# tnwei/waternet

Measured on NVIDIA H100. Metric: images/sec at 1080p batch16 (preprocess + gated-fusion forward, uint8 in -> uint8 out), higher is better.
Workload: dtype bf16 + fp8 corrections (v = hi + lo: hi x hi in bf16, both correction terms of the heavy layers as one e4m3 MMA; fp32 accumulate; 3-term bf16 elsewhere)

## Files before the change

### waternet_b200/csrc/common.cuh

```cuda
#pragma once

#include <cuda_runtime.h>
#include <stdint.h>
#include <stdio.h>

#include "../../include/waternet_b200.h"
#include "tiling.cuh"

namespace wn {

void set_error(const char* fmt, ...);

#define WN_CUDA(call)                                                                   \
  do {                                                                                  \
    cudaError_t err__ = (call);                                                         \
    if (err__ != cudaSuccess) {                                                         \
      wn::set_error("%s:%d: %s -> %s", __FILE__, __LINE__, #call, cudaGetErrorString(err__)); \
      return WN_E_CUDA;                                                                 \
    }                                                                                   \
  } while (0)

#define WN_LAUNCH_CHECK(h)   \
  do {                       \
    (h)->launches++;         \
// ... 144 lines not shown
};
struct FwdOpts {
  int scheme = 0;
  int dbg_layer = -1;
  float* dbg_dst = nullptr;
  bool packed = false;
  bool hi_only = false;
  const int* run_if = nullptr;
  uint8_t* out_u8 = nullptr;
  PeerOut peers = {};
  int stack = kStackAll;
  bool refiner_l1 = false;
  const TileGeom* tiles = nullptr;
  long long win0 = 0;
  const RaggedWindow* rwin = nullptr;
};
int umma_forward_layers(wn_handle* h, const float* const in[4], const int64_t st[4][4], float* out, int n,
                        int height, int width, const FwdBuffers& b, cudaStream_t stream,
                        const FwdOpts& opts = FwdOpts());
int umma_debug_layer(wn_handle* h, const float* const in[4], const int64_t in_strides[4][4], int n,
                     int height, int width, int layer, float* dst, void* workspace,
                     size_t workspace_bytes, cudaStream_t stream, int scheme = 0);
int umma_pack_weights(wn_handle* h, const float* const* params, cudaStream_t stream);
void umma_free(wn_handle* h);
size_t umma_forward_workspace_bytes(int n, int h, int w);
int umma_chunk_images(const wn_handle* h, int n, int height, int width);
int umma_forward(wn_handle* h, const float* const in[4], const int64_t in_strides[4][4], float* out,
                 int n, int height, int width, void* workspace, size_t workspace_bytes,
                 cudaStream_t stream, int scheme = 0, int stack = kStackAll, float* refined = nullptr);
size_t umma_forward_tiled_workspace_bytes(int n, int h, int w, int tile_h, int tile_w, long long max_pass_pixels,
// ... 51 lines not shown
```

### waternet_b200/csrc/conv_umma.cu

```cuda
#include "umma_conv.cuh"

namespace wn {

struct PackInArgs {
  const float* p[4];
  long long s[4][4];
};
enum PackForm { kPackImages = 0, kPackWindows = 1, kPackFlag = 2 };
template <int FORM = kPackImages>
__global__ void __launch_bounds__(256) pack_inputs_kernel(PackInArgs a, uint4* __restrict__ out, int H, int W,
                                                          int* __restrict__ exact_flag, TileGeom tiles, long long win0) {
  const int pix = blockIdx.x * 256 + threadIdx.x;
  const int hw = FORM == kPackWindows ? tiles.win_h * tiles.win_w : H * W;
  bool exact = true;
  if (pix < hw) {
    int n = blockIdx.y, y, x;
    if constexpr (FORM == kPackWindows) {
      const TileWindow t = tile_window(tiles, win0 + blockIdx.y);
      const int wy = pix / tiles.win_w;
      n = t.img;
      y = t.ys + wy;
      x = t.xs + (pix - wy * tiles.win_w);
    } else {
      y = pix / W;
// ... 59 lines not shown
static constexpr UmmaLayerSpec kSpecs[kNumUmmaLayers] = {
    {7, 16, 224, kEpiAct, 0, 1, 1, 0, false, 1, 1},
    {5, 128, 128, kEpiAct, 0, 1, 5, 1, true, 1, 1},
    {3, 128, 128, kEpiAct, 0, 1, 3, 2, true, 1, 1},
    {1, 128, 64, kEpiAct, 1, 1, 1, 3, false, 1, 1},
    {7, 64, 64, kEpiAct, 1, 1, 7, 4, true, 2, 1},
    {5, 64, 64, kEpiAct, 1, 1, 5, 5, true, 2, 1},
    {3, 64, 64, kEpiAct, 1, 1, 9, 6, true, 2, 1},
    {3, 64, 16, kEpiSigmoid, 1, 1, 9, 7, false, 1, 1},
    {5, 96, 32, kEpiAct, 1, 3, 5, 9, true, 1, 1},
    {3, 96, 16, kEpiGate, 1, 1, 9, 10, false, 1, 1},
    {7, 16, 96, kEpiAct, 0, 1, 1, 8, false, 1, 1}};

static_assert(kSpecs[kC2].f8 == kSpecs[kR2].f8, "L1 writes one format for both of its consumers");
static constexpr bool writes_f8(int li) { return li < kR3 && li != kC8 && kSpecs[li + 1].f8; }

static __global__ void __launch_bounds__(256)
mirror_u8_kernel(const uint8_t* __restrict__ src, PeerOut peers, size_t bytes, const int* __restrict__ run_if) {
  if (run_if && *run_if == 0) return;
  const size_t stride = (size_t)gridDim.x * blockDim.x, i0 = (size_t)blockIdx.x * blockDim.x + threadIdx.x;
#pragma unroll
  for (int k = 0; k < WN_MAX_PEERS; k++) {
    if (k >= peers.n) continue;
    uint8_t* dst = peers.p[k];
    const size_t vecs = (((reinterpret_cast<uintptr_t>(src) | reinterpret_cast<uintptr_t>(dst)) & 15) == 0) ? bytes / 16 : 0;
    for (size_t i = i0; i < vecs; i += stride) reinterpret_cast<uint4*>(dst)[i] = reinterpret_cast<const uint4*>(src)[i];
    for (size_t i = vecs * 16 + i0; i < bytes; i += stride) dst[i] = src[i];
  }
}
int mirror_u8(wn_handle* h, const uint8_t* src, const PeerOut& peers, size_t bytes, const int* run_if, cudaStream_t stream) {
// ... 109 lines not shown
  if (cap <= 0 || cap > kDefaultChunkPixels) cap = kDefaultChunkPixels;
  long long per = (long long)h * w;
  long long nb = cap / (per > 0 ? per : 1);
  if (nb < 1) nb = 1;
  return nb < n ? (int)nb : n;
}
int umma_chunk_images(const wn_handle* h, int n, int height, int width) {
  return umma_chunk(h ? h->chunk_pixels : 0, n, height, width);
}

size_t umma_forward_workspace_bytes(int n, int h, int w) {
  const size_t nb = (size_t)umma_chunk(0, n, h, w);
  return nb * h * w * kUmmaBytesPerPixel + nb * h * 64 + 4096;
}

template <int LI, bool RAG>
static int launch_layer_as(wn_handle* h, bool f8, void* in_base, ConvArgs a, cudaStream_t stream) {
  constexpr UmmaLayerSpec s = kSpecs[LI];
  constexpr bool R = RAG && s.epi != kEpiSigmoid;
  const UmmaWeights* u = h->umma;
  constexpr int GW = s.npad / s.ng;
  if (f8) {
    constexpr int FMT = (s.f8 ? kFmtIn8 : 0) | (writes_f8(LI) ? kFmtOut8 : 0);
    if constexpr ((FMT & kFmtOut8) != 0) a.f8_overflow = u->overflow_dev;
    if constexpr (s.f8) a.f8_scale = u->scale8[LI] + 1;
    return launch_conv<s.ks, s.cinpad, GW, s.epi, (s.f8 ? 0 : s.concat), s.nblk, s.tps, FMT, R, s.mw, s.ng>(
        h, s.slot, s.f8 ? u->stages8[LI] : u->stages[LI], u->bias[LI], in_base, a, stream);
  }
  return launch_conv<s.ks, s.cinpad, GW, s.epi, s.concat, s.nblk, s.tps, 0, R, s.mw, s.ng>(
      h, s.slot, u->stages[LI], u->bias[LI], in_base, a, stream);
}
template <int LI>
static int launch_layer(wn_handle* h, bool f8, void* in_base, ConvArgs a, cudaStream_t stream) {
  return a.rwin ? launch_layer_as<LI, true>(h, f8, in_base, a, stream)
                : launch_layer_as<LI, false>(h, f8, in_base, a, stream);
}

__global__ void decode_planes_kernel(const uint4* __restrict__ src, float* __restrict__ dst, int planes_half, int hw,
                                     int f8) {
  const int n = blockIdx.z, plane = blockIdx.y;
  const int pix = blockIdx.x * blockDim.x + threadIdx.x;
  if (pix >= hw) return;
  const uint4 h4 = src[((size_t)n * 2 * planes_half + plane) * hw + pix];
  if (f8) {
    const uint4 l4 = src[((size_t)n * 2 * planes_half + planes_half + 2 * (plane >> 1)) * hw + pix];
    const uint32_t hs[4] = {h4.x, h4.y, h4.z, h4.w}, ls[4] = {l4.x, l4.y, l4.z, l4.w};
#pragma unroll
    for (int j = 0; j < 8; j++) {
      const float hi = __uint_as_float(((hs[j >> 1] >> ((j & 1) * 16)) & 0xffffu) << 16);
      const int byte = (plane & 1) * 8 + j;
// ... 76 lines not shown
    act(b.r[1], 96, nullptr, 0);
    rc = launch_conv<s.ks, s.cinpad, s.npad, s.epi, s.concat, s.nblk, s.tps, 0, false, s.mw, s.ng>(
        h, s.slot, h->umma->stages[kRL1], h->umma->bias[kRL1], b.act0, a, stream);
    if (rc) return rc;
  } else {
    act(b.a[1], 128, b.r[1], b.r[1] ? 96 : 0);
    if ((rc = launch_layer<kL1>(h, f8, b.act0, a, stream))) return rc;
  }
  a.skip_lo = nullptr;
  a.a_hi_only = 0;
  if (dump(kL1)) return WN_OK;
  if (want_cmg) {
    act(b.a[2], 128, nullptr, 0);
    if ((rc = launch_layer<kC2>(h, f8, b.a[1], a, stream))) return rc;
    if (dump(kC2)) return WN_OK;
    act(b.a[3], 128, nullptr, 0);
    if ((rc = launch_layer<kC3>(h, f8, b.a[2], a, stream))) return rc;
    if (dump(kC3)) return WN_OK;
    act(b.a[4], 64, nullptr, 0);
    if ((rc = launch_layer<kC4>(h, f8, b.a[3], a, stream))) return rc;
    if (dump(kC4)) return WN_OK;
    act(b.a[5], 64, nullptr, 0);
    if ((rc = launch_layer<kC5>(h, f8, b.a[4], a, stream))) return rc;
    if (dump(kC5)) return WN_OK;
    act(b.a[6], 64, nullptr, 0);
    if ((rc = launch_layer<kC6>(h, f8, b.a[5], a, stream))) return rc;
    if (dump(kC6)) return WN_OK;
    act(b.a[7], 64, nullptr, 0);
    if ((rc = launch_layer<kC7>(h, f8, b.a[6], a, stream))) return rc;
    if (dump(kC7)) return WN_OK;
    const bool dump_maps = dbg_layer == kSpecs[kC8].slot;
    a.out_f32 = dump_maps ? dbg_dst : b.cm;
    if ((rc = launch_layer<kC8>(h, f8, b.a[7], a, stream))) return rc;
    if (dump_maps) return WN_OK;
  }
// ... 16 lines not shown

static FwdBuffers carve(void* workspace, int n, int H, int W) {
  const size_t px = (size_t)n * H * W;
  uint8_t* ws = (uint8_t*)(((uintptr_t)workspace + 1023) / 1024 * 1024);
  uint4* cmgAB[2];
  uint4* refAB[2];
  FwdBuffers b;
  memset(&b, 0, sizeof(b));
  b.act0 = (uint4*)ws;     ws += px * 64;
  cmgAB[0] = (uint4*)ws;   ws += px * 512;
  cmgAB[1] = (uint4*)ws;   ws += px * 512;
  refAB[0] = (uint4*)ws;   ws += px * 384;
  refAB[1] = (uint4*)ws;   ws += px * 384;
  b.cm = (float*)ws;       ws += px * 12;
  b.exact_flag = (int*)(((uintptr_t)ws + 255) / 256 * 256);
  for (int l = 1; l <= 7; l++) b.a[l] = cmgAB[(l - 1) & 1];
  b.r[1] = refAB[0];
  b.r[2] = refAB[1];
  return b;
}

static int umma_pass(wn_handle* h, const float* const in[4], const int64_t st[4][4], float* out, int n, int H, int W,
                     const FwdBuffers& b, cudaStream_t stream, FwdOpts o) {
  int rc = umma_forward_layers(h, in, st, out, n, H, W, b, stream, o);
  if (rc || o.scheme != 1 || o.dbg_layer >= 0) return rc;
  o.scheme = 0;
  o.packed = true;
  o.run_if = h->umma->overflow_dev;
  Timing* timing = h->timing;
  h->timing = nullptr;
  rc = umma_forward_layers(h, in, st, out, n, H, W, b, stream, o);
  h->timing = timing;
  return rc;
}

int umma_debug_layer(wn_handle* h, const float* const in[4], const int64_t in_strides[4][4], int n, int H, int W,
                     int layer, float* dst, void* workspace, size_t workspace_bytes, cudaStream_t stream, int scheme) {
  if (!h->umma || umma_chunk(0, n, H, W) != n || workspace_bytes < umma_forward_workspace_bytes(n, H, W)) {
    set_error("debug layer dump: weights not packed, batch too large for one pass or workspace too small");
    return WN_E_WORKSPACE;
  }
  int rc = get_encoder();
  if (rc) return rc;
  FwdOpts o;
  o.scheme = scheme;
  o.dbg_layer = layer;
  o.dbg_dst = dst;
  return umma_forward_layers(h, in, in_strides, nullptr, n, H, W, carve(workspace, n, H, W), stream, o);
}

static int effective_scheme(wn_handle* h, int scheme) {
  return (scheme == 1 && *h->umma->overflow_host) ? 0 : scheme;
}
static int mirror_overflow(wn_handle* h, int scheme, cudaStream_t stream) {
  if (scheme == 1)
    WN_CUDA(cudaMemcpyAsync(h->umma->overflow_host, h->umma->overflow_dev, sizeof(int), cudaMemcpyDeviceToHost, stream));
  return WN_OK;
}

int umma_forward(wn_handle* h, const float* const in[4], const int64_t in_strides[4][4], float* out, int n, int H,
                 int W, void* workspace, size_t workspace_bytes, cudaStream_t stream, int scheme, int stack,
                 float* refined) {
// ... 298 lines not shown
```

### waternet_b200/csrc/umma_conv.cuh

```cuda
#pragma once

#include <cuda.h>
#include <cuda_bf16.h>

#include "common.cuh"
#include "wgmma_ops.cuh"

namespace wn {

__device__ __forceinline__ uint32_t smem_u32(const void* p) {
  return (uint32_t)__cvta_generic_to_shared(p);
}
__device__ __forceinline__ void mbar_init(uint64_t* bar, uint32_t count) {
  asm volatile("mbarrier.init.shared::cta.b64 [%0], %1;" ::"r"(smem_u32(bar)), "r"(count));
}
__device__ __forceinline__ void mbar_wait(uint64_t* bar, uint32_t parity) {
  for (uint32_t it = 0; it < (1u << 26); it++) {
    uint32_t done;
    asm volatile(
        "{\n\t.reg .pred p;\n\t"
        "mbarrier.try_wait.parity.shared::cta.b64 p, [%1], %2;\n\t"
        "selp.u32 %0, 1, 0, p;\n\t}"
        : "=r"(done)
        : "r"(smem_u32(bar)), "r"(parity)
// ... 42 lines not shown
  uint16_t v;
  asm("cvt.rn.satfinite.e4m3x2.f32 %0, %1, %2;" : "=h"(v) : "f"(f1), "f"(f0));
  return v;
}

enum Epilogue { kEpiAct = 0, kEpiSigmoid = 1, kEpiGate = 2, kEpiDgrad = 3 };

constexpr int kTileH = 16;
constexpr int kThreads = 320;
constexpr int kWarpA = 8, kWarpB = 9;
constexpr int kConsumerWarps = 8;
constexpr int kStageLd = 36;

constexpr int kFmtIn8 = 1, kFmtOut8 = 2;
template <int KS, int CIN_PAD, int NPAD, int CONCAT = 0, int NBLK = 1, int TPS = 1, int FMT = 0, int MW = 1,
          int NG = 1>
struct UmmaCfg {
  static constexpr bool F8IN = (FMT & kFmtIn8) != 0;
  static constexpr bool DUAL = CONCAT != 0;
  static constexpr int TILE_W = 8 * MW;
  static constexpr int HALO_W = TILE_W + KS - 1, HALO_H = kTileH + KS - 1;
  static constexpr int NCHUNK = CIN_PAD / 16;
  static constexpr int PLANE_BYTES = HALO_W * HALO_H * 16;
  static constexpr int A_STAGE = (4 * PLANE_BYTES + 1023) / 1024 * 1024;
  static constexpr int B_TAP = NPAD * 64;
  static constexpr int B_STAGE = TPS * B_TAP;
  static_assert((KS * KS) % TPS == 0, "taps per weight stage must divide the filter");
  static constexpr int NSTAGE_PER_CHUNK = KS * KS / TPS;
  static constexpr int STAGING = 2 * 64 * kStageLd * 4;
  static constexpr int BUDGET = 227 * 1024 - 1024 - 2048 - STAGING;
  static constexpr int NA_WANT = NCHUNK == 1 ? 2 : KS == 1 ? 6 : 3;
  static constexpr int NB_FIT = (BUDGET - NA_WANT * A_STAGE) / B_STAGE;
  static constexpr int NB = NB_FIT > 8 ? 8 : NB_FIT < 2 ? 2 : NB_FIT;
  static constexpr int NA_FIT = (BUDGET - NB * B_STAGE) / A_STAGE;
  static constexpr int NA = NA_FIT > NA_WANT ? NA_WANT : NA_FIT;
  static_assert(!F8IN || !CONCAT, "fp8 corrections: the [hi | second part] weight layout");
  static constexpr int CPB = NCHUNK / NBLK;
  static constexpr int BLK_COLS = DUAL ? 2 * NPAD : NPAD;
  static constexpr int COLS = NBLK * BLK_COLS;
  static constexpr int ACC = COLS / 2;
  static constexpr int ACC8 = F8IN ? ACC : 1;
  static constexpr int SMEM_BYTES = NA * A_STAGE + NB * B_STAGE + STAGING + 2048 + 1024;
  static_assert(NA >= 1, "halo tile does not fit in shared memory");
  static_assert(NCHUNK % NBLK == 0, "chunks must split evenly over the diagonal blocks");
  static_assert(NPAD % 16 == 0 && (DUAL ? 2 : 1) * NPAD <= 256, "invalid wgmma N");
  static_assert(MW == 1 || MW == 2, "one or two m64 blocks per warpgroup");
  static_assert(NG == 1 || NBLK == 1, "column groups of a block-diagonal layer");
  static_assert(MW * (ACC + (F8IN ? ACC8 : 0)) <= 128, "accumulators do not fit in registers");
  static constexpr size_t GROUP_BYTES = (size_t)NCHUNK * NSTAGE_PER_CHUNK * B_STAGE;
};

struct ActDst {
  uint4* base;
  int planes_half;
};

struct ConvArgs {
  const uint8_t* wpk;
  const float* bias;
  int N, H, W;
  int in_planes_half;
  int tiles_x, tiles_y;
  ActDst dst0, dst1;
  int split_c;
// ... 1 lines not shown
  float* out_f32;
  const float* cm;
  uint8_t* out_u8;
  const int* skip_lo;
  int a_hi_only;
  float* refined_out;
  const uint4* mask_base;
  int mask_planes_half;
  const float* f8_scale;
  int* f8_overflow;
  const int* run_if;
  int tiled;
  long long win0;
  TileGeom tiles;
  const RaggedWindow* rwin;
};

__device__ __forceinline__ uint32_t pack_bf16x2(__nv_bfloat16 a, __nv_bfloat16 b) {
  return (uint32_t)__bfloat16_as_ushort(a) | ((uint32_t)__bfloat16_as_ushort(b) << 16);
}
__device__ __forceinline__ void split_bf16x2(float f0, float f1, uint32_t& hi, uint32_t& lo) {
  const __nv_bfloat162 h = __floats2bfloat162_rn(f0, f1);
  hi = *reinterpret_cast<const uint32_t*>(&h);
  const float h0 = __uint_as_float(hi << 16), h1 = __uint_as_float(hi & 0xffff0000u);
  const __nv_bfloat162 l = __floats2bfloat162_rn(f0 - h0, f1 - h1);
  lo = *reinterpret_cast<const uint32_t*>(&l);
}

template <int EPI, bool OUT8, bool RAG = false>
__device__ __forceinline__ void epilogue16(const ConvArgs& g, const float* s_bias, const float* f, int ch, int n,
// ... 116 lines not shown
        if (out_f32) {
#pragma unroll
          for (int c = 0; c < 3; c++) out_f32[oo + c * ohw] = v[c];
        }
        if (out_u8) {
          uint8_t* q = out_u8 + o8;
#pragma unroll
          for (int c = 0; c < 3; c++) q[c] = (uint8_t)(int)__fmul_rn(fminf(fmaxf(v[c], 0.0f), 1.0f), 255.0f);
        }
      }
    }
  }
}

template <int KS, int CIN_PAD, int NPAD, int EPI, int CONCAT, int NBLK, int TPS, int FMT = 0, bool RAG = false,
          int MW = 1, int NG = 1>
__global__ void __launch_bounds__(kThreads, 1)
conv_umma_kernel(const __grid_constant__ CUtensorMap tmap_in, const ConvArgs g) {
  using C = UmmaCfg<KS, CIN_PAD, NPAD, CONCAT, NBLK, TPS, FMT, MW, NG>;
  constexpr bool F8IN = C::F8IN, DUAL = C::DUAL, OUT8 = (FMT & kFmtOut8) != 0;
  static_assert(!OUT8 || EPI == kEpiAct, "fp8 planes are written by the activation epilogue only");
  static_assert(!RAG || EPI == kEpiAct || EPI == kEpiGate, "ragged passes mask activations and store the gate");
  if (g.run_if != nullptr && *reinterpret_cast<const volatile int*>(g.run_if) == 0) return;
  extern __shared__ uint8_t smem_raw[];
  uint8_t* smem = reinterpret_cast<uint8_t*>((reinterpret_cast<uintptr_t>(smem_raw) + 1023) & ~(uintptr_t)1023);
  uint8_t* a_stages = smem;
  uint8_t* b_stages = smem + C::NA * C::A_STAGE;
  float* staging = reinterpret_cast<float*>(b_stages + C::NB * C::B_STAGE);
  uint8_t* tail = reinterpret_cast<uint8_t*>(staging) + C::STAGING;
  uint64_t* a_full = reinterpret_cast<uint64_t*>(tail);
  uint64_t* a_empty = a_full + C::NA;
  uint64_t* b_full = a_empty + C::NA;
  uint64_t* b_empty = b_full + C::NB;
  float* s_bias = reinterpret_cast<float*>(tail + 512);
  static_assert((2 * 6 + 2 * 8) * 8 <= 512 && NG * NBLK * NPAD * 4 <= 2048 - 512, "barrier / bias area");

  const int tid = threadIdx.x, warp = tid >> 5, lane = tid & 31;
  const int num_tiles = g.tiles_x * g.tiles_y * g.N * NG;
  if (tid == 0) {
    for (int i = 0; i < C::NA; i++) { mbar_init(&a_full[i], 1); mbar_init(&a_empty[i], kConsumerWarps); }
    for (int i = 0; i < C::NB; i++) { mbar_init(&b_full[i], 1); mbar_init(&b_empty[i], kConsumerWarps); }
    asm volatile("fence.mbarrier_init.release.cluster;" ::: "memory");
  }
  for (int i = tid; i < NG * NBLK * NPAD; i += kThreads) s_bias[i] = g.bias[i];
  __syncthreads();

  if (warp == kWarpA) {
    if (lane == 0) {
      int stage = 0;
      uint32_t phase = 0;
      for (int tile = blockIdx.x; tile < num_tiles; tile += gridDim.x) {
        const int pt = tile / NG;
        const int n = pt / (g.tiles_x * g.tiles_y);
        const int rem = pt - n * g.tiles_x * g.tiles_y;
        const int ty = rem / g.tiles_x, tx = rem - ty * g.tiles_x;
        const int x0 = tx * C::TILE_W - KS / 2, y0 = ty * kTileH - KS / 2;
        for (int c = 0; c < C::NCHUNK; c++) {
          mbar_wait(&a_empty[stage], phase ^ 1);
          uint8_t* dst = a_stages + stage * C::A_STAGE;
          mbar_expect_tx(&a_full[stage], (g.a_hi_only ? 2 : 4) * C::PLANE_BYTES);
          tma_load_5d(dst, &tmap_in, &a_full[stage], 0, x0, y0, 2 * c, n);
          if (!g.a_hi_only)
            tma_load_5d(dst + 2 * C::PLANE_BYTES, &tmap_in, &a_full[stage], 0, x0, y0, g.in_planes_half + 2 * c, n);
          if (++stage == C::NA) { stage = 0; phase ^= 1; }
        }
      }
    }
    return;
  }
  if (warp == kWarpB) {
    if (lane == 0) {
      int stage = 0;
      uint32_t phase = 0;
      for (int tile = blockIdx.x; tile < num_tiles; tile += gridDim.x) {
        const uint8_t* wpk = g.wpk + (size_t)(tile % NG) * C::GROUP_BYTES;
        for (int it = 0; it < C::NCHUNK * C::NSTAGE_PER_CHUNK; it++) {
          mbar_wait(&b_empty[stage], phase ^ 1);
          mbar_expect_tx(&b_full[stage], C::B_STAGE);
          bulk_load(b_stages + stage * C::B_STAGE, wpk + (size_t)it * C::B_STAGE, C::B_STAGE, &b_full[stage]);
          if (++stage == C::NB) { stage = 0; phase ^= 1; }
        }
      }
    }
    return;
  }

// ... 63 lines not shown
        wg_wait<1>();
        release();
        pend_b = bstage;
        if (tg == C::NSTAGE_PER_CHUNK - 1) pend_a = astage;
        if (++bstage == C::NB) { bstage = 0; bphase ^= 1; }
      }
      if (++astage == C::NA) { astage = 0; aphase ^= 1; }
    }
    wg_wait<0>();
    release();

    const int pt = tile / NG, c0 = (tile % NG) * NPAD;
    const int n = pt / (g.tiles_x * g.tiles_y);
    const int rem = pt - n * g.tiles_x * g.tiles_y;
    const int ty = rem / g.tiles_x, tx = rem - ty * g.tiles_x;
    float* stg = staging + wg * 64 * kStageLd;
    const int frow = (warp & 3) * 16 + (lane >> 2), fcol = (lane & 3) * 2;
    const int r = wtid & 63, half = wtid >> 6;
    const int m = wg * 64 + r;
    const int gy = ty * kTileH + (m >> 3);
    constexpr int NCH = NBLK * NPAD;
#pragma unroll
    for (int mb = 0; mb < MW; mb++) {
      const int gx = tx * C::TILE_W + mb * 8 + (m & 7);
      const bool inside = gx < g.W && gy < g.H;
      bool valid = true;
      if constexpr (RAG) valid = gx < g.rwin[n].vw && gy < g.rwin[n].vh;
#pragma unroll
      for (int ch0 = 0; ch0 < NCH; ch0 += 32) {
#pragma unroll
        for (int j = 0; j < 4; j++) {
          const int ch = ch0 + 8 * j;
          if (ch < NCH) {
            const int col = NBLK > 1 ? (ch / NPAD) * C::BLK_COLS + ch % NPAD : ch;
            float v[4];
#pragma unroll
            for (int k = 0; k < 4; k++) {
              v[k] = acc[mb][col / 2 + k];
              if constexpr (DUAL) v[k] += acc[mb][(col + NPAD) / 2 + k];
              if constexpr (F8IN) v[k] = (v[k] + acc8[mb][col / 2 + k]) * dscale;
            }
            float* s = stg + frow * kStageLd + 8 * j + fcol;
            *reinterpret_cast<float2*>(s) = make_float2(v[0], v[1]);
            *reinterpret_cast<float2*>(s + 8 * kStageLd) = make_float2(v[2], v[3]);
          }
        }
        wg_bar(1 + wg);
        const int cb = ch0 + 16 * half;
        if (cb < NCH && inside) {
          float f[16];
          const float4* s = reinterpret_cast<const float4*>(stg + r * kStageLd + 16 * half);
#pragma unroll
          for (int q = 0; q < 4; q++) {
            const float4 x = s[q];
            f[4 * q] = x.x; f[4 * q + 1] = x.y; f[4 * q + 2] = x.z; f[4 * q + 3] = x.w;
          }
          epilogue16<EPI, OUT8, RAG>(g, s_bias, f, c0 + cb, n, gx, gy, valid);
        }
        wg_bar(1 + wg);
      }
    }
  }
}

static __global__ void scatter_weights_kernel(const float* __restrict__ src, float* __restrict__ dense, int co, int ci,
                                       int kk, int cinpad, int row_off, int split, int base0, int base1,
                                       float divisor) {
  const int total = co * ci * kk;
  for (int i = blockIdx.x * blockDim.x + threadIdx.x; i < total; i += gridDim.x * blockDim.x) {
    int t = i % kk;
    int c = (i / kk) % ci;
    int o = i / (kk * ci);
// ... 112 lines not shown
  cuuint64_t strides[4] = {16, (cuuint64_t)W * 16, (cuuint64_t)H * W * 16, (cuuint64_t)planes_total * H * W * 16};
  cuuint32_t box[5] = {8, (cuuint32_t)halo_w, (cuuint32_t)halo_h, 2, 1};
  cuuint32_t estr[5] = {1, 1, 1, 1, 1};
  CUresult r = g_encode(tm, CU_TENSOR_MAP_DATA_TYPE_BFLOAT16, 5, base, dims, strides, box, estr,
                        CU_TENSOR_MAP_INTERLEAVE_NONE, CU_TENSOR_MAP_SWIZZLE_NONE, CU_TENSOR_MAP_L2_PROMOTION_L2_128B,
                        CU_TENSOR_MAP_FLOAT_OOB_FILL_NONE);
  if (r != CUDA_SUCCESS) {
    set_error("cuTensorMapEncodeTiled failed with %d (planes=%d N=%d H=%d W=%d box=%dx%d)", (int)r, planes_total, N, H,
              W, halo_w, halo_h);
    return WN_E_CUDA;
  }
  return WN_OK;
}

template <int KS, int CIN_PAD, int NPAD, int EPI, int CONCAT = 0, int NBLK = 1, int TPS = 1, int FMT = 0,
          bool RAG = false, int MW = 1, int NG = 1>
static int launch_conv(wn_handle* h, int slot, const uint8_t* wpk, const float* bias, void* in_base, ConvArgs a,
                       cudaStream_t stream) {
  using C = UmmaCfg<KS, CIN_PAD, NPAD, CONCAT, NBLK, TPS, FMT, MW, NG>;
  int rc = get_encoder();
  if (rc) return rc;
  CUtensorMap tm;
  rc = make_tmap(&tm, in_base, (a.a_hi_only ? 1 : 2) * (CIN_PAD / 8), a.N, a.H, a.W, C::HALO_W, C::HALO_H);
  if (rc) return rc;
  a.wpk = wpk;
  a.bias = bias;
  a.in_planes_half = CIN_PAD / 8;
  a.tiles_x = (a.W + C::TILE_W - 1) / C::TILE_W;
  a.tiles_y = (a.H + kTileH - 1) / kTileH;
  const long long tiles = (long long)a.tiles_x * a.tiles_y * a.N * NG;
  auto kern = conv_umma_kernel<KS, CIN_PAD, NPAD, EPI, CONCAT, NBLK, TPS, FMT, RAG, MW, NG>;
  WN_CUDA(cudaFuncSetAttribute(kern, cudaFuncAttributeMaxDynamicSharedMemorySize, C::SMEM_BYTES));
  TimedScope ts(h, slot, stream);
  const int grid = (int)(tiles < h->sm_count ? tiles : h->sm_count);
  kern<<<grid, kThreads, C::SMEM_BYTES, stream>>>(tm, a);
  WN_LAUNCH_CHECK(h);
  return WN_OK;
}

}
```

### waternet_b200/csrc/wgmma_ops.cuh

```cuda
#pragma once

#include <stdint.h>

namespace wn {

template <int N>
__device__ __forceinline__ void wgmma_bf16(float* d, uint64_t da, uint64_t db) {
  if constexpr (N == 16) {
    asm volatile("{\n\t.reg .pred p;\n\tsetp.ne.b32 p, 1, 0;\n\t"
                 "wgmma.mma_async.sync.aligned.m64n16k16.f32.bf16.bf16 {%0, %1, %2, %3, %4, %5, %6, %7}, %8, %9, p, 1, 1, 0, 0;\n\t}"
                 : "+f"(d[0]), "+f"(d[1]), "+f"(d[2]), "+f"(d[3]), "+f"(d[4]), "+f"(d[5]), "+f"(d[6]), "+f"(d[7])
                 : "l"(da), "l"(db));
  } else if constexpr (N == 32) {
    asm volatile("{\n\t.reg .pred p;\n\tsetp.ne.b32 p, 1, 0;\n\t"
                 "wgmma.mma_async.sync.aligned.m64n32k16.f32.bf16.bf16 {%0, %1, %2, %3, %4, %5, %6, %7, %8, %9, %10, %11, %12, %13, %14, %15}, %16, %17, p, 1, 1, 0, 0;\n\t}"
                 : "+f"(d[0]), "+f"(d[1]), "+f"(d[2]), "+f"(d[3]), "+f"(d[4]), "+f"(d[5]), "+f"(d[6]), "+f"(d[7]), "+f"(d[8]), "+f"(d[9]), "+f"(d[10]), "+f"(d[11]), "+f"(d[12]), "+f"(d[13]), "+f"(d[14]), "+f"(d[15])
                 : "l"(da), "l"(db));
  } else if constexpr (N == 64) {
    asm volatile("{\n\t.reg .pred p;\n\tsetp.ne.b32 p, 1, 0;\n\t"
                 "wgmma.mma_async.sync.aligned.m64n64k16.f32.bf16.bf16 {%0, %1, %2, %3, %4, %5, %6, %7, %8, %9, %10, %11, %12, %13, %14, %15, %16, %17, %18, %19, %20, %21, %22, %23, %24, %25, %26, %27, %28, %29, %30, %31}, %32, %33, p, 1, 1, 0, 0;\n\t}"
                 : "+f"(d[0]), "+f"(d[1]), "+f"(d[2]), "+f"(d[3]), "+f"(d[4]), "+f"(d[5]), "+f"(d[6]), "+f"(d[7]), "+f"(d[8]), "+f"(d[9]), "+f"(d[10]), "+f"(d[11]), "+f"(d[12]), "+f"(d[13]), "+f"(d[14]), "+f"(d[15]), "+f"(d[16]), "+f"(d[17]), "+f"(d[18]), "+f"(d[19]), "+f"(d[20]), "+f"(d[21]), "+f"(d[22]), "+f"(d[23]), "+f"(d[24]), "+f"(d[25]), "+f"(d[26]), "+f"(d[27]), "+f"(d[28]), "+f"(d[29]), "+f"(d[30]), "+f"(d[31])
                 : "l"(da), "l"(db));
  } else if constexpr (N == 96) {
    asm volatile("{\n\t.reg .pred p;\n\tsetp.ne.b32 p, 1, 0;\n\t"
// ... 36 lines not shown
    asm volatile("{\n\t.reg .pred p;\n\tsetp.ne.b32 p, 1, 0;\n\t"
                 "wgmma.mma_async.sync.aligned.m64n96k16.f32.bf16.bf16 {%0, %1, %2, %3, %4, %5, %6, %7, %8, %9, %10, %11, %12, %13, %14, %15, %16, %17, %18, %19, %20, %21, %22, %23, %24, %25, %26, %27, %28, %29, %30, %31, %32, %33, %34, %35, %36, %37, %38, %39, %40, %41, %42, %43, %44, %45, %46, %47}, %48, %49, p, 1, 1, 1, 1;\n\t}"
                 : "+f"(d[0]), "+f"(d[1]), "+f"(d[2]), "+f"(d[3]), "+f"(d[4]), "+f"(d[5]), "+f"(d[6]), "+f"(d[7]), "+f"(d[8]), "+f"(d[9]), "+f"(d[10]), "+f"(d[11]), "+f"(d[12]), "+f"(d[13]), "+f"(d[14]), "+f"(d[15]), "+f"(d[16]), "+f"(d[17]), "+f"(d[18]), "+f"(d[19]), "+f"(d[20]), "+f"(d[21]), "+f"(d[22]), "+f"(d[23]), "+f"(d[24]), "+f"(d[25]), "+f"(d[26]), "+f"(d[27]), "+f"(d[28]), "+f"(d[29]), "+f"(d[30]), "+f"(d[31]), "+f"(d[32]), "+f"(d[33]), "+f"(d[34]), "+f"(d[35]), "+f"(d[36]), "+f"(d[37]), "+f"(d[38]), "+f"(d[39]), "+f"(d[40]), "+f"(d[41]), "+f"(d[42]), "+f"(d[43]), "+f"(d[44]), "+f"(d[45]), "+f"(d[46]), "+f"(d[47])
                 : "l"(da), "l"(db));
  } else if constexpr (N == 128) {
    asm volatile("{\n\t.reg .pred p;\n\tsetp.ne.b32 p, 1, 0;\n\t"
                 "wgmma.mma_async.sync.aligned.m64n128k16.f32.bf16.bf16 {%0, %1, %2, %3, %4, %5, %6, %7, %8, %9, %10, %11, %12, %13, %14, %15, %16, %17, %18, %19, %20, %21, %22, %23, %24, %25, %26, %27, %28, %29, %30, %31, %32, %33, %34, %35, %36, %37, %38, %39, %40, %41, %42, %43, %44, %45, %46, %47, %48, %49, %50, %51, %52, %53, %54, %55, %56, %57, %58, %59, %60, %61, %62, %63}, %64, %65, p, 1, 1, 1, 1;\n\t}"
                 : "+f"(d[0]), "+f"(d[1]), "+f"(d[2]), "+f"(d[3]), "+f"(d[4]), "+f"(d[5]), "+f"(d[6]), "+f"(d[7]), "+f"(d[8]), "+f"(d[9]), "+f"(d[10]), "+f"(d[11]), "+f"(d[12]), "+f"(d[13]), "+f"(d[14]), "+f"(d[15]), "+f"(d[16]), "+f"(d[17]), "+f"(d[18]), "+f"(d[19]), "+f"(d[20]), "+f"(d[21]), "+f"(d[22]), "+f"(d[23]), "+f"(d[24]), "+f"(d[25]), "+f"(d[26]), "+f"(d[27]), "+f"(d[28]), "+f"(d[29]), "+f"(d[30]), "+f"(d[31]), "+f"(d[32]), "+f"(d[33]), "+f"(d[34]), "+f"(d[35]), "+f"(d[36]), "+f"(d[37]), "+f"(d[38]), "+f"(d[39]), "+f"(d[40]), "+f"(d[41]), "+f"(d[42]), "+f"(d[43]), "+f"(d[44]), "+f"(d[45]), "+f"(d[46]), "+f"(d[47]), "+f"(d[48]), "+f"(d[49]), "+f"(d[50]), "+f"(d[51]), "+f"(d[52]), "+f"(d[53]), "+f"(d[54]), "+f"(d[55]), "+f"(d[56]), "+f"(d[57]), "+f"(d[58]), "+f"(d[59]), "+f"(d[60]), "+f"(d[61]), "+f"(d[62]), "+f"(d[63])
                 : "l"(da), "l"(db));
  } else {
    static_assert(N < 0, "wgmma shape not generated (tools/gen_wgmma.py)");
  }
}

template <int N>
__device__ __forceinline__ void wgmma_e4m3(float* d, uint64_t da, uint64_t db) {
  if constexpr (N == 32) {
    asm volatile("{\n\t.reg .pred p;\n\tsetp.ne.b32 p, 1, 0;\n\t"
                 "wgmma.mma_async.sync.aligned.m64n32k32.f32.e4m3.e4m3 {%0, %1, %2, %3, %4, %5, %6, %7, %8, %9, %10, %11, %12, %13, %14, %15}, %16, %17, p, 1, 1;\n\t}"
                 : "+f"(d[0]), "+f"(d[1]), "+f"(d[2]), "+f"(d[3]), "+f"(d[4]), "+f"(d[5]), "+f"(d[6]), "+f"(d[7]), "+f"(d[8]), "+f"(d[9]), "+f"(d[10]), "+f"(d[11]), "+f"(d[12]), "+f"(d[13]), "+f"(d[14]), "+f"(d[15])
                 : "l"(da), "l"(db));
  } else if constexpr (N == 64) {
    asm volatile("{\n\t.reg .pred p;\n\tsetp.ne.b32 p, 1, 0;\n\t"
                 "wgmma.mma_async.sync.aligned.m64n64k32.f32.e4m3.e4m3 {%0, %1, %2, %3, %4, %5, %6, %7, %8, %9, %10, %11, %12, %13, %14, %15, %16, %17, %18, %19, %20, %21, %22, %23, %24, %25, %26, %27, %28, %29, %30, %31}, %32, %33, p, 1, 1;\n\t}"
                 : "+f"(d[0]), "+f"(d[1]), "+f"(d[2]), "+f"(d[3]), "+f"(d[4]), "+f"(d[5]), "+f"(d[6]), "+f"(d[7]), "+f"(d[8]), "+f"(d[9]), "+f"(d[10]), "+f"(d[11]), "+f"(d[12]), "+f"(d[13]), "+f"(d[14]), "+f"(d[15]), "+f"(d[16]), "+f"(d[17]), "+f"(d[18]), "+f"(d[19]), "+f"(d[20]), "+f"(d[21]), "+f"(d[22]), "+f"(d[23]), "+f"(d[24]), "+f"(d[25]), "+f"(d[26]), "+f"(d[27]), "+f"(d[28]), "+f"(d[29]), "+f"(d[30]), "+f"(d[31])
                 : "l"(da), "l"(db));
  } else if constexpr (N == 128) {
    asm volatile("{\n\t.reg .pred p;\n\tsetp.ne.b32 p, 1, 0;\n\t"
                 "wgmma.mma_async.sync.aligned.m64n128k32.f32.e4m3.e4m3 {%0, %1, %2, %3, %4, %5, %6, %7, %8, %9, %10, %11, %12, %13, %14, %15, %16, %17, %18, %19, %20, %21, %22, %23, %24, %25, %26, %27, %28, %29, %30, %31, %32, %33, %34, %35, %36, %37, %38, %39, %40, %41, %42, %43, %44, %45, %46, %47, %48, %49, %50, %51, %52, %53, %54, %55, %56, %57, %58, %59, %60, %61, %62, %63}, %64, %65, p, 1, 1;\n\t}"
                 : "+f"(d[0]), "+f"(d[1]), "+f"(d[2]), "+f"(d[3]), "+f"(d[4]), "+f"(d[5]), "+f"(d[6]), "+f"(d[7]), "+f"(d[8]), "+f"(d[9]), "+f"(d[10]), "+f"(d[11]), "+f"(d[12]), "+f"(d[13]), "+f"(d[14]), "+f"(d[15]), "+f"(d[16]), "+f"(d[17]), "+f"(d[18]), "+f"(d[19]), "+f"(d[20]), "+f"(d[21]), "+f"(d[22]), "+f"(d[23]), "+f"(d[24]), "+f"(d[25]), "+f"(d[26]), "+f"(d[27]), "+f"(d[28]), "+f"(d[29]), "+f"(d[30]), "+f"(d[31]), "+f"(d[32]), "+f"(d[33]), "+f"(d[34]), "+f"(d[35]), "+f"(d[36]), "+f"(d[37]), "+f"(d[38]), "+f"(d[39]), "+f"(d[40]), "+f"(d[41]), "+f"(d[42]), "+f"(d[43]), "+f"(d[44]), "+f"(d[45]), "+f"(d[46]), "+f"(d[47]), "+f"(d[48]), "+f"(d[49]), "+f"(d[50]), "+f"(d[51]), "+f"(d[52]), "+f"(d[53]), "+f"(d[54]), "+f"(d[55]), "+f"(d[56]), "+f"(d[57]), "+f"(d[58]), "+f"(d[59]), "+f"(d[60]), "+f"(d[61]), "+f"(d[62]), "+f"(d[63])
// ... 8 lines not shown
```

Before: 51.61.

## Fuse the 1x1 C4 conv into C3's epilogue via register-sourced wgmma

C3's accumulator is activated, split into bf16 hi/lo register fragments and fed directly into a register-A wgmma against C4's weights, which are held in shared memory for the whole kernel. C4's output is then written by the normal epilogue. This removes the separate C4 launch and the round trip of C3's 128-channel activation through global memory. In exchange C3 gets less shared memory for pipeline stages (fewer A stages with fp8 input) and more register pressure, and the buffer assignment changes so C3 writes straight into C4's slot.

```diff
diff --git a/waternet_b200/csrc/common.cuh b/waternet_b200/csrc/common.cuh
--- a/waternet_b200/csrc/common.cuh
+++ b/waternet_b200/csrc/common.cuh
@@ -182,6 +182,7 @@
   const TileGeom* tiles = nullptr;
   long long win0 = 0;
   const RaggedWindow* rwin = nullptr;
+  bool fuse_c4 = false;
 };
 int umma_forward_layers(wn_handle* h, const float* const in[4], const int64_t st[4][4], float* out, int n,
                         int height, int width, const FwdBuffers& b, cudaStream_t stream,
diff --git a/waternet_b200/csrc/conv_umma.cu b/waternet_b200/csrc/conv_umma.cu
--- a/waternet_b200/csrc/conv_umma.cu
+++ b/waternet_b200/csrc/conv_umma.cu
@@ -97,6 +97,13 @@
 
 static_assert(kSpecs[kC2].f8 == kSpecs[kR2].f8, "L1 writes one format for both of its consumers");
 static constexpr bool writes_f8(int li) { return li < kR3 && li != kC8 && kSpecs[li + 1].f8; }
+
+static_assert(kSpecs[kC4].ks == 1 && kSpecs[kC4].cinpad == kSpecs[kC3].npad && kSpecs[kC4].epi == kEpiAct &&
+                  kSpecs[kC4].concat && kSpecs[kC4].nblk == 1 && !kSpecs[kC4].f8 && kSpecs[kC4].mw == 1 &&
+                  kSpecs[kC4].ng == 1 && kSpecs[kC3].mw == 1 && kSpecs[kC3].ng == 1 && !writes_f8(kC3),
+              "C4 fuses into C3 as a 1x1 bf16x3 CONCAT layer on 8 x 16-pixel tiles");
+static_assert(FusedCfg<kSpecs[kC3].npad, kSpecs[kC4].npad>::W_BYTES ==
+                  (kSpecs[kC4].cinpad / 16) * kSpecs[kC4].npad * 64, "C4's packed weight image is resident as a whole");
 
 static __global__ void __launch_bounds__(256)
 mirror_u8_kernel(const uint8_t* __restrict__ src, PeerOut peers, size_t bytes, const int* __restrict__ run_if) {
@@ -236,26 +243,32 @@
   return nb * h * w * kUmmaBytesPerPixel + nb * h * 64 + 4096;
 }
 
-template <int LI, bool RAG>
+template <int LI, bool RAG, bool FUSED = false>
 static int launch_layer_as(wn_handle* h, bool f8, void* in_base, ConvArgs a, cudaStream_t stream) {
   constexpr UmmaLayerSpec s = kSpecs[LI];
+  static_assert(!FUSED || LI == kC3, "only C4 fuses, behind C3");
+  constexpr int FUSE = FUSED ? kSpecs[kC4].npad : 0;
   constexpr bool R = RAG && s.epi != kEpiSigmoid;
   const UmmaWeights* u = h->umma;
   constexpr int GW = s.npad / s.ng;
+  if constexpr (FUSED) {
+    a.fuse_wpk = u->stages[kC4];
+    a.fuse_bias = u->bias[kC4];
+  }
   if (f8) {
-    constexpr int FMT = (s.f8 ? kFmtIn8 : 0) | (writes_f8(LI) ? kFmtOut8 : 0);
+    constexpr int FMT = (s.f8 ? kFmtIn8 : 0) | (writes_f8(FUSED ? kC4 : LI) ? kFmtOut8 : 0);
     if constexpr ((FMT & kFmtOut8) != 0) a.f8_overflow = u->overflow_dev;
     if constexpr (s.f8) a.f8_scale = u->scale8[LI] + 1;
-    return launch_conv<s.ks, s.cinpad, GW, s.epi, (s.f8 ? 0 : s.concat), s.nblk, s.tps, FMT, R, s.mw, s.ng>(
+    return launch_conv<s.ks, s.cinpad, GW, s.epi, (s.f8 ? 0 : s.concat), s.nblk, s.tps, FMT, R, s.mw, s.ng, FUSE>(
         h, s.slot, s.f8 ? u->stages8[LI] : u->stages[LI], u->bias[LI], in_base, a, stream);
   }
-  return launch_conv<s.ks, s.cinpad, GW, s.epi, s.concat, s.nblk, s.tps, 0, R, s.mw, s.ng>(
+  return launch_conv<s.ks, s.cinpad, GW, s.epi, s.concat, s.nblk, s.tps, 0, R, s.mw, s.ng, FUSE>(
       h, s.slot, u->stages[LI], u->bias[LI], in_base, a, stream);
 }
-template <int LI>
+template <int LI, bool FUSED = false>
 static int launch_layer(wn_handle* h, bool f8, void* in_base, ConvArgs a, cudaStream_t stream) {
-  return a.rwin ? launch_layer_as<LI, true>(h, f8, in_base, a, stream)
-                : launch_layer_as<LI, false>(h, f8, in_base, a, stream);
+  return a.rwin ? launch_layer_as<LI, true, FUSED>(h, f8, in_base, a, stream)
+                : launch_layer_as<LI, false, FUSED>(h, f8, in_base, a, stream);
 }
 
 __global__ void decode_planes_kernel(const uint4* __restrict__ src, float* __restrict__ dst, int planes_half, int hw,
@@ -362,11 +375,20 @@
     act(b.a[2], 128, nullptr, 0);
     if ((rc = launch_layer<kC2>(h, f8, b.a[1], a, stream))) return rc;
     if (dump(kC2)) return WN_OK;
-    act(b.a[3], 128, nullptr, 0);
-    if ((rc = launch_layer<kC3>(h, f8, b.a[2], a, stream))) return rc;
-    if (dump(kC3)) return WN_OK;
-    act(b.a[4], 64, nullptr, 0);
-    if ((rc = launch_layer<kC4>(h, f8, b.a[3], a, stream))) return rc;
+    if (o.fuse_c4 && dbg_layer != kSpecs[kC3].slot) {
+      act(b.a[4], 64, nullptr, 0);
+      if ((rc = launch_layer<kC3, true>(h, f8, b.a[2], a, stream))) return rc;
+    } else {
+      act(b.a[3], 128, nullptr, 0);
+      if ((rc = launch_layer<kC3>(h, f8, b.a[2], a, stream))) return rc;
+      if (dump(kC3)) return WN_OK;
+      if (b.a[3] == b.a[4]) {
+        set_error("C4 as a launch of its own needs a buffer for C3's output");
+        return WN_E_STATE;
+      }
+      act(b.a[4], 64, nullptr, 0);
+      if ((rc = launch_layer<kC4>(h, f8, b.a[3], a, stream))) return rc;
+    }
     if (dump(kC4)) return WN_OK;
     act(b.a[5], 64, nullptr, 0);
     if ((rc = launch_layer<kC5>(h, f8, b.a[4], a, stream))) return rc;
@@ -413,7 +435,7 @@
   refAB[1] = (uint4*)ws;   ws += px * 384;
   b.cm = (float*)ws;       ws += px * 12;
   b.exact_flag = (int*)(((uintptr_t)ws + 255) / 256 * 256);
-  for (int l = 1; l <= 7; l++) b.a[l] = cmgAB[(l - 1) & 1];
+  for (int l = 1; l <= 7; l++) b.a[l] = cmgAB[(l - (l >= 4 ? 0 : 1)) & 1];
   b.r[1] = refAB[0];
   b.r[2] = refAB[1];
   return b;
@@ -421,6 +443,7 @@
 
 static int umma_pass(wn_handle* h, const float* const in[4], const int64_t st[4][4], float* out, int n, int H, int W,
                      const FwdBuffers& b, cudaStream_t stream, FwdOpts o) {
+  o.fuse_c4 = true;
   int rc = umma_forward_layers(h, in, st, out, n, H, W, b, stream, o);
   if (rc || o.scheme != 1 || o.dbg_layer >= 0) return rc;
   o.scheme = 0;
@@ -445,6 +468,7 @@
   o.scheme = scheme;
   o.dbg_layer = layer;
   o.dbg_dst = dst;
+  o.fuse_c4 = true;
   return umma_forward_layers(h, in, in_strides, nullptr, n, H, W, carve(workspace, n, H, W), stream, o);
 }
 
diff --git a/waternet_b200/csrc/umma_conv.cuh b/waternet_b200/csrc/umma_conv.cuh
--- a/waternet_b200/csrc/umma_conv.cuh
+++ b/waternet_b200/csrc/umma_conv.cuh
@@ -80,7 +80,7 @@
 
 constexpr int kFmtIn8 = 1, kFmtOut8 = 2;
 template <int KS, int CIN_PAD, int NPAD, int CONCAT = 0, int NBLK = 1, int TPS = 1, int FMT = 0, int MW = 1,
-          int NG = 1>
+          int NG = 1, int RES = 0>
 struct UmmaCfg {
   static constexpr bool F8IN = (FMT & kFmtIn8) != 0;
   static constexpr bool DUAL = CONCAT != 0;
@@ -94,8 +94,8 @@
   static_assert((KS * KS) % TPS == 0, "taps per weight stage must divide the filter");
   static constexpr int NSTAGE_PER_CHUNK = KS * KS / TPS;
   static constexpr int STAGING = 2 * 64 * kStageLd * 4;
-  static constexpr int BUDGET = 227 * 1024 - 1024 - 2048 - STAGING;
-  static constexpr int NA_WANT = NCHUNK == 1 ? 2 : KS == 1 ? 6 : 3;
+  static constexpr int BUDGET = 227 * 1024 - 1024 - 2048 - STAGING - RES;
+  static constexpr int NA_WANT = NCHUNK == 1 ? 2 : KS == 1 ? 6 : (RES && (FMT & 1)) ? 2 : 3;
   static constexpr int NB_FIT = (BUDGET - NA_WANT * A_STAGE) / B_STAGE;
   static constexpr int NB = NB_FIT > 8 ? 8 : NB_FIT < 2 ? 2 : NB_FIT;
   static constexpr int NA_FIT = (BUDGET - NB * B_STAGE) / A_STAGE;
@@ -106,7 +106,7 @@
   static constexpr int COLS = NBLK * BLK_COLS;
   static constexpr int ACC = COLS / 2;
   static constexpr int ACC8 = F8IN ? ACC : 1;
-  static constexpr int SMEM_BYTES = NA * A_STAGE + NB * B_STAGE + STAGING + 2048 + 1024;
+  static constexpr int SMEM_BYTES = NA * A_STAGE + NB * B_STAGE + RES + STAGING + 2048 + 1024;
   static_assert(NA >= 1, "halo tile does not fit in shared memory");
   static_assert(NCHUNK % NBLK == 0, "chunks must split evenly over the diagonal blocks");
   static_assert(NPAD % 16 == 0 && (DUAL ? 2 : 1) * NPAD <= 256, "invalid wgmma N");
@@ -114,6 +114,14 @@
   static_assert(NG == 1 || NBLK == 1, "column groups of a block-diagonal layer");
   static_assert(MW * (ACC + (F8IN ? ACC8 : 0)) <= 128, "accumulators do not fit in registers");
   static constexpr size_t GROUP_BYTES = (size_t)NCHUNK * NSTAGE_PER_CHUNK * B_STAGE;
+};
+
+template <int CIN, int NOUT>
+struct FusedCfg {
+  static constexpr int KC = CIN / 16;
+  static constexpr int CHUNK_BYTES = NOUT * 64;
+  static constexpr int W_BYTES = KC * CHUNK_BYTES;
+  static constexpr int ACC = NOUT;
 };
 
 struct ActDst {
@@ -145,6 +153,8 @@
   long long win0;
   TileGeom tiles;
   const RaggedWindow* rwin;
+  const uint8_t* fuse_wpk;
+  const float* fuse_bias;
 };
 
 __device__ __forceinline__ uint32_t pack_bf16x2(__nv_bfloat16 a, __nv_bfloat16 b) {
@@ -291,35 +301,43 @@
 }
 
 template <int KS, int CIN_PAD, int NPAD, int EPI, int CONCAT, int NBLK, int TPS, int FMT = 0, bool RAG = false,
-          int MW = 1, int NG = 1>
+          int MW = 1, int NG = 1, int FUSE = 0>
 __global__ void __launch_bounds__(kThreads, 1)
 conv_umma_kernel(const __grid_constant__ CUtensorMap tmap_in, const ConvArgs g) {
-  using C = UmmaCfg<KS, CIN_PAD, NPAD, CONCAT, NBLK, TPS, FMT, MW, NG>;
+  using F = FusedCfg<NPAD, FUSE>;
+  using C = UmmaCfg<KS, CIN_PAD, NPAD, CONCAT, NBLK, TPS, FMT, MW, NG, FUSE ? F::W_BYTES : 0>;
   constexpr bool F8IN = C::F8IN, DUAL = C::DUAL, OUT8 = (FMT & kFmtOut8) != 0;
   static_assert(!OUT8 || EPI == kEpiAct, "fp8 planes are written by the activation epilogue only");
   static_assert(!RAG || EPI == kEpiAct || EPI == kEpiGate, "ragged passes mask activations and store the gate");
+  static_assert(!FUSE || (EPI == kEpiAct && MW == 1 && NG == 1 && NBLK == 1 && !DUAL && F::ACC == C::ACC),
+                "a fused layer reads one plain activation accumulator of 8 x 16-pixel tiles and takes its registers");
   if (g.run_if != nullptr && *reinterpret_cast<const volatile int*>(g.run_if) == 0) return;
   extern __shared__ uint8_t smem_raw[];
   uint8_t* smem = reinterpret_cast<uint8_t*>((reinterpret_cast<uintptr_t>(smem_raw) + 1023) & ~(uintptr_t)1023);
   uint8_t* a_stages = smem;
   uint8_t* b_stages = smem + C::NA * C::A_STAGE;
-  float* staging = reinterpret_cast<float*>(b_stages + C::NB * C::B_STAGE);
+  uint8_t* w_fused = b_stages + C::NB * C::B_STAGE;
+  float* staging = reinterpret_cast<float*>(w_fused + (FUSE ? F::W_BYTES : 0));
   uint8_t* tail = reinterpret_cast<uint8_t*>(staging) + C::STAGING;
   uint64_t* a_full = reinterpret_cast<uint64_t*>(tail);
   uint64_t* a_empty = a_full + C::NA;
   uint64_t* b_full = a_empty + C::NA;
   uint64_t* b_empty = b_full + C::NB;
+  uint64_t* w_full = b_empty + C::NB;
   float* s_bias = reinterpret_cast<float*>(tail + 512);
-  static_assert((2 * 6 + 2 * 8) * 8 <= 512 && NG * NBLK * NPAD * 4 <= 2048 - 512, "barrier / bias area");
+  static_assert((2 * 6 + 2 * 8 + 1) * 8 <= 512 && (NG * NBLK * NPAD + FUSE) * 4 <= 2048 - 512, "barrier / bias area");
 
   const int tid = threadIdx.x, warp = tid >> 5, lane = tid & 31;
   const int num_tiles = g.tiles_x * g.tiles_y * g.N * NG;
   if (tid == 0) {
     for (int i = 0; i < C::NA; i++) { mbar_init(&a_full[i], 1); mbar_init(&a_empty[i], kConsumerWarps); }
     for (int i = 0; i < C::NB; i++) { mbar_init(&b_full[i], 1); mbar_init(&b_empty[i], kConsumerWarps); }
+    if constexpr (FUSE != 0) mbar_init(w_full, 1);
     asm volatile("fence.mbarrier_init.release.cluster;" ::: "memory");
   }
   for (int i = tid; i < NG * NBLK * NPAD; i += kThreads) s_bias[i] = g.bias[i];
+  if constexpr (FUSE != 0)
+    for (int i = tid; i < FUSE; i += kThreads) s_bias[NPAD + i] = g.fuse_bias[i];
   __syncthreads();
 
   if (warp == kWarpA) {
@@ -347,6 +365,10 @@
   }
   if (warp == kWarpB) {
     if (lane == 0) {
+      if constexpr (FUSE != 0) {
+        mbar_expect_tx(w_full, F::W_BYTES);
+        bulk_load(w_fused, g.fuse_wpk, F::W_BYTES, w_full);
+      }
       int stage = 0;
       uint32_t phase = 0;
       for (int tile = blockIdx.x; tile < num_tiles; tile += gridDim.x) {
@@ -440,12 +462,63 @@
     const int n = pt / (g.tiles_x * g.tiles_y);
     const int rem = pt - n * g.tiles_x * g.tiles_y;
     const int ty = rem / g.tiles_x, tx = rem - ty * g.tiles_x;
+    const int frow = (warp & 3) * 16 + (lane >> 2), fcol = (lane & 3) * 2;
+    if constexpr (FUSE != 0) {
+      bool valid[2] = {true, true};
+      if constexpr (RAG) {
+        const int m = wg * 64 + frow;
+        const int gx = tx * C::TILE_W + (m & 7), gy = ty * kTileH + (m >> 3);
+        valid[0] = gx < g.rwin[n].vw && gy < g.rwin[n].vh;
+        valid[1] = gx < g.rwin[n].vw && gy + 1 < g.rwin[n].vh;
+      }
+      uint32_t a_hi[F::KC][4], a_lo[F::KC][4];
+#pragma unroll
+      for (int kc = 0; kc < F::KC; kc++) {
+#pragma unroll
+        for (int q = 0; q < 4; q++) {
+          const int i = 8 * kc + 2 * q, ch = 16 * kc + 8 * (q >> 1) + fcol;
+          float f[2];
+#pragma unroll
+          for (int e = 0; e < 2; e++) {
+            float v = acc[0][i + e];
+            if constexpr (F8IN) v = __fmul_rn(v + acc8[0][i + e], dscale);
+            v = fmaxf(v + s_bias[ch + e], 0.f);
+            if constexpr (RAG) v = valid[q & 1] ? v : 0.f;
+            f[e] = v;
+          }
+          split_bf16x2(f[0], f[1], a_hi[kc][q], a_lo[kc][q]);
+        }
+      }
+#pragma unroll
+      for (int i = 0; i < C::ACC; i++) acc[0][i] = 0.f;
+      mbar_wait(w_full, 0);
+      const uint32_t w_base = smem_u32(w_fused);
+      wg_fence();
+#pragma unroll
+      for (int kc = 0; kc < F::KC; kc++) {
+        const uint64_t b = make_desc(w_base + kc * F::CHUNK_BYTES, 2 * FUSE * 16, 128);
+        wgmma_bf16_rs<2 * FUSE>(acc[0], a_hi[kc], b);
+        wgmma_bf16_rs<FUSE>(acc[0], a_lo[kc], b);
+      }
+      wg_commit();
+      wg_wait<0>();
+#pragma unroll
+      for (int kc = 0; kc < F::KC; kc++)
+#pragma unroll
+        for (int q = 0; q < 4; q++) asm volatile("" : "+r"(a_hi[kc][q]), "+r"(a_lo[kc][q]));
+#pragma unroll
+      for (int i = 0; i < C::ACC; i++) asm volatile("" : "+f"(acc[0][i]));
+    }
+
+    constexpr int E_NPAD = FUSE ? FUSE : NPAD;
+    constexpr bool E_DUAL = FUSE ? true : DUAL, E_F8IN = FUSE ? false : F8IN;
+    constexpr int E_BLK_COLS = E_DUAL ? 2 * E_NPAD : E_NPAD;
+    const float* e_bias = FUSE ? s_bias + NPAD : s_bias;
     float* stg = staging + wg * 64 * kStageLd;
-    const int frow = (warp & 3) * 16 + (lane >> 2), fcol = (lane & 3) * 2;
     const int r = wtid & 63, half = wtid >> 6;
     const int m = wg * 64 + r;
     const int gy = ty * kTileH + (m >> 3);
-    constexpr int NCH = NBLK * NPAD;
+    constexpr int NCH = NBLK * E_NPAD;
 #pragma unroll
     for (int mb = 0; mb < MW; mb++) {
       const int gx = tx * C::TILE_W + mb * 8 + (m & 7);
@@ -458,13 +531,13 @@
         for (int j = 0; j < 4; j++) {
           const int ch = ch0 + 8 * j;
           if (ch < NCH) {
-            const int col = NBLK > 1 ? (ch / NPAD) * C::BLK_COLS + ch % NPAD : ch;
+            const int col = NBLK > 1 ? (ch / E_NPAD) * E_BLK_COLS + ch % E_NPAD : ch;
             float v[4];
 #pragma unroll
             for (int k = 0; k < 4; k++) {
               v[k] = acc[mb][col / 2 + k];
-              if constexpr (DUAL) v[k] += acc[mb][(col + NPAD) / 2 + k];
-              if constexpr (F8IN) v[k] = (v[k] + acc8[mb][col / 2 + k]) * dscale;
+              if constexpr (E_DUAL) v[k] += acc[mb][(col + E_NPAD) / 2 + k];
+              if constexpr (E_F8IN) v[k] = (v[k] + acc8[mb][col / 2 + k]) * dscale;
             }
             float* s = stg + frow * kStageLd + 8 * j + fcol;
             *reinterpret_cast<float2*>(s) = make_float2(v[0], v[1]);
@@ -481,7 +554,7 @@
             const float4 x = s[q];
             f[4 * q] = x.x; f[4 * q + 1] = x.y; f[4 * q + 2] = x.z; f[4 * q + 3] = x.w;
           }
-          epilogue16<EPI, OUT8, RAG>(g, s_bias, f, c0 + cb, n, gx, gy, valid);
+          epilogue16<EPI, OUT8, RAG>(g, e_bias, f, c0 + cb, n, gx, gy, valid);
         }
         wg_bar(1 + wg);
       }
@@ -624,10 +697,10 @@
 }
 
 template <int KS, int CIN_PAD, int NPAD, int EPI, int CONCAT = 0, int NBLK = 1, int TPS = 1, int FMT = 0,
-          bool RAG = false, int MW = 1, int NG = 1>
+          bool RAG = false, int MW = 1, int NG = 1, int FUSE = 0>
 static int launch_conv(wn_handle* h, int slot, const uint8_t* wpk, const float* bias, void* in_base, ConvArgs a,
                        cudaStream_t stream) {
-  using C = UmmaCfg<KS, CIN_PAD, NPAD, CONCAT, NBLK, TPS, FMT, MW, NG>;
+  using C = UmmaCfg<KS, CIN_PAD, NPAD, CONCAT, NBLK, TPS, FMT, MW, NG, FUSE ? FusedCfg<NPAD, FUSE>::W_BYTES : 0>;
   int rc = get_encoder();
   if (rc) return rc;
   CUtensorMap tm;
@@ -639,7 +712,7 @@
   a.tiles_x = (a.W + C::TILE_W - 1) / C::TILE_W;
   a.tiles_y = (a.H + kTileH - 1) / kTileH;
   const long long tiles = (long long)a.tiles_x * a.tiles_y * a.N * NG;
-  auto kern = conv_umma_kernel<KS, CIN_PAD, NPAD, EPI, CONCAT, NBLK, TPS, FMT, RAG, MW, NG>;
+  auto kern = conv_umma_kernel<KS, CIN_PAD, NPAD, EPI, CONCAT, NBLK, TPS, FMT, RAG, MW, NG, FUSE>;
   WN_CUDA(cudaFuncSetAttribute(kern, cudaFuncAttributeMaxDynamicSharedMemorySize, C::SMEM_BYTES));
   TimedScope ts(h, slot, stream);
   const int grid = (int)(tiles < h->sm_count ? tiles : h->sm_count);
diff --git a/waternet_b200/csrc/wgmma_ops.cuh b/waternet_b200/csrc/wgmma_ops.cuh
--- a/waternet_b200/csrc/wgmma_ops.cuh
+++ b/waternet_b200/csrc/wgmma_ops.cuh
@@ -74,6 +74,23 @@
 }
 
 template <int N>
+__device__ __forceinline__ void wgmma_bf16_rs(float* d, const uint32_t* a, uint64_t db) {
+  if constexpr (N == 64) {
+    asm volatile("{\n\t.reg .pred p;\n\tsetp.ne.b32 p, 1, 0;\n\t"
+                 "wgmma.mma_async.sync.aligned.m64n64k16.f32.bf16.bf16 {%0, %1, %2, %3, %4, %5, %6, %7, %8, %9, %10, %11, %12, %13, %14, %15, %16, %17, %18, %19, %20, %21, %22, %23, %24, %25, %26, %27, %28, %29, %30, %31}, {%32, %33, %34, %35}, %36, p, 1, 1, 0;\n\t}"
+                 : "+f"(d[0]), "+f"(d[1]), "+f"(d[2]), "+f"(d[3]), "+f"(d[4]), "+f"(d[5]), "+f"(d[6]), "+f"(d[7]), "+f"(d[8]), "+f"(d[9]), "+f"(d[10]), "+f"(d[11]), "+f"(d[12]), "+f"(d[13]), "+f"(d[14]), "+f"(d[15]), "+f"(d[16]), "+f"(d[17]), "+f"(d[18]), "+f"(d[19]), "+f"(d[20]), "+f"(d[21]), "+f"(d[22]), "+f"(d[23]), "+f"(d[24]), "+f"(d[25]), "+f"(d[26]), "+f"(d[27]), "+f"(d[28]), "+f"(d[29]), "+f"(d[30]), "+f"(d[31])
+                 : "r"(a[0]), "r"(a[1]), "r"(a[2]), "r"(a[3]), "l"(db));
+  } else if constexpr (N == 128) {
+    asm volatile("{\n\t.reg .pred p;\n\tsetp.ne.b32 p, 1, 0;\n\t"
+                 "wgmma.mma_async.sync.aligned.m64n128k16.f32.bf16.bf16 {%0, %1, %2, %3, %4, %5, %6, %7, %8, %9, %10, %11, %12, %13, %14, %15, %16, %17, %18, %19, %20, %21, %22, %23, %24, %25, %26, %27, %28, %29, %30, %31, %32, %33, %34, %35, %36, %37, %38, %39, %40, %41, %42, %43, %44, %45, %46, %47, %48, %49, %50, %51, %52, %53, %54, %55, %56, %57, %58, %59, %60, %61, %62, %63}, {%64, %65, %66, %67}, %68, p, 1, 1, 0;\n\t}"
+                 : "+f"(d[0]), "+f"(d[1]), "+f"(d[2]), "+f"(d[3]), "+f"(d[4]), "+f"(d[5]), "+f"(d[6]), "+f"(d[7]), "+f"(d[8]), "+f"(d[9]), "+f"(d[10]), "+f"(d[11]), "+f"(d[12]), "+f"(d[13]), "+f"(d[14]), "+f"(d[15]), "+f"(d[16]), "+f"(d[17]), "+f"(d[18]), "+f"(d[19]), "+f"(d[20]), "+f"(d[21]), "+f"(d[22]), "+f"(d[23]), "+f"(d[24]), "+f"(d[25]), "+f"(d[26]), "+f"(d[27]), "+f"(d[28]), "+f"(d[29]), "+f"(d[30]), "+f"(d[31]), "+f"(d[32]), "+f"(d[33]), "+f"(d[34]), "+f"(d[35]), "+f"(d[36]), "+f"(d[37]), "+f"(d[38]), "+f"(d[39]), "+f"(d[40]), "+f"(d[41]), "+f"(d[42]), "+f"(d[43]), "+f"(d[44]), "+f"(d[45]), "+f"(d[46]), "+f"(d[47]), "+f"(d[48]), "+f"(d[49]), "+f"(d[50]), "+f"(d[51]), "+f"(d[52]), "+f"(d[53]), "+f"(d[54]), "+f"(d[55]), "+f"(d[56]), "+f"(d[57]), "+f"(d[58]), "+f"(d[59]), "+f"(d[60]), "+f"(d[61]), "+f"(d[62]), "+f"(d[63])
+                 : "r"(a[0]), "r"(a[1]), "r"(a[2]), "r"(a[3]), "l"(db));
+  } else {
+    static_assert(N < 0, "wgmma shape not generated (tools/gen_wgmma.py)");
+  }
+}
+
+template <int N>
 __device__ __forceinline__ void wgmma_e4m3(float* d, uint64_t da, uint64_t db) {
   if constexpr (N == 32) {
     asm volatile("{\n\t.reg .pred p;\n\tsetp.ne.b32 p, 1, 0;\n\t"
```

New measurement: 53.38 (median of 6 runs). +3.4%, better.
